# MGI-tech-bioinformatics/SuperPlus

Measured on AMD Instinct MI355X. Metric: k-mers/s (DF createDict stage: trim + canonical k-mer count + solid filter + spectrum + adjacency), higher is better.
Workload: dtype u64

## Files before the change

### superplus_amd/csrc/dfk.hip

```cpp
#include "../../include/dfk.h"
#include "dfk_kernels.h"
#include "dfk_arena.h"

#include <algorithm>
#include <chrono>
#include <cstdarg>
#include <cstdio>
#include <cstdlib>
#include <cstring>
#include <atomic>
#include <fcntl.h>
#include <functional>
#include <new>
#include <string>
#include <sys/mman.h>
#include <sys/stat.h>
#include <unistd.h>
#include <condition_variable>
#include <memory>
#include <mutex>
#include <numeric>
#include <thread>
#include <vector>

// ... 70 lines not shown
    void release(DevBuf& b) { arena.release(b); }
    void shrink(DevBuf& b, size_t keep) { arena.shrink(b, keep); }
    void release_since(uint64_t mark, const DevBuf* keep = nullptr) { arena.release_since(mark, keep); }
    uint64_t largest_allocatable() const { return arena.largest_allocatable(); }
    void drop_empty_chunks() { arena.drop_empty_chunks(); }
    void drop_pool() { arena.drop_pool(); }
    bool have = false;
    uint64_t n_reads = 0;
    struct FileRange { const char* base; uint64_t bytes; int fd; uint64_t off; };
    std::vector<FileRange> file_ranges;
    DevBuf good_len;
    struct Part { DevBuf buf, pre; uint64_t n = 0; uint64_t blist = 0, n_blist = 0; bool listed = false; };
    bool want_blist = false;
    int pending_blist = -1;
    std::function<int()> after_count_launch;
    std::vector<Part> parts;
    uint64_t n_solid = 0, n_boundary = 0;
    unsigned seg_attempt = 0;
    double distinct_per_inst = 0.0;
    double plan_derate = 0.95;
    std::vector<int64_t> hist;
    std::vector<dfk_entry32> sorted, sorted_pre;
    bool sorted_ok = false, sorted_pre_ok = false;
    dfk_stats st{};
    bool shard_open = false, shard_use_bc = false;
    const void* sh_in[7] = {};
    uint64_t sh_packed_bytes = 0, sh_pq_bytes = 0, sh_n_reads = 0, sh_n_inst_local = 0;
    int64_t sh_read_id0 = 0;
    DevBuf shard_send[2];
    uint32_t shard_send_pass[2] = {~0u, ~0u};
// ... 8 lines not shown
    uint32_t shard_world = 1, shard_log2_nb = 0;
    void* shard_state = nullptr;
    void (*shard_state_free)(void*) = nullptr;
    void* lane_pool = nullptr; void (*lane_pool_free)(void*) = nullptr;
    std::mutex lane_mu;
    void* graph_state = nullptr;
    void (*graph_state_free)(void*) = nullptr;
    unsigned int* d_resident = nullptr;
    unsigned int resident_target = 0;
    unsigned int last_wg_idle = 0;
    void* kept[6] = {};
    uint64_t kept_packed_bytes = 0, kept_pq_bytes = 0, kept_n_reads = 0, kept_budget = 0;

    void release_all()
    {
        after_count_launch = nullptr;
        if (stream2) (void)hipStreamSynchronize(stream2);
        DevBuf* live[] = {&good_len, &shard_send[0], &shard_send[1], &shard_recv[0], &shard_recv[1], &adj_keys, &adj_src, &set};
        for (DevBuf* d : live) release(*d);
        for (Part& pt : parts) { release(pt.buf); release(pt.pre); }
        parts.clear();
        arena.reset();
        good_len = shard_send[0] = shard_send[1] = shard_recv[0] = shard_recv[1] = adj_keys = adj_src = set = DevBuf{};
        shard_send_pass[0] = shard_send_pass[1] = ~0u;
        have = false; sorted_ok = sorted_pre_ok = false; sorted.clear(); sorted_pre.clear(); hist.clear();
        n_solid = 0; adj_n = 0; shard_open = false;
        if (shard_state) { shard_state_free(shard_state); shard_state = nullptr; }
        for (void*& p : sh_staged) if (p) { (void)hipFree(p); p = nullptr; }
        budget += budget_taken; budget_taken = 0;
        if (graph_state) { graph_state_free(graph_state); graph_state = nullptr; }
    }
    void drop_kept()
// ... 10 lines not shown
            if (i < 5 && b >= (64ull << 20) && ((uintptr_t)kept[i] & 0xFFF) == 0) arena.adopt(kept[i], b);
            else (void)hipFree(kept[i]);
            kept[i] = nullptr;
        }
        budget += kept_budget; kept_budget = 0; kept_n_reads = 0;
    }
};

namespace {

struct Timer {
    hipEvent_t a{}, b{}; hipStream_t s;
    explicit Timer(hipStream_t st) : s(st) { (void)hipEventCreate(&a); (void)hipEventCreate(&b); }
    ~Timer() { (void)hipEventDestroy(a); (void)hipEventDestroy(b); }
    void start() { (void)hipEventRecord(a, s); }
    float stop() { (void)hipEventRecord(b, s); (void)hipEventSynchronize(b); float ms = 0; (void)hipEventElapsedTime(&ms, a, b); return ms; }
};

template <int K>
int stage_trim(dfk_ctx* c, const Inputs& in, uint64_t* n_inst)
{
    DevBuf ctr; int rc = c->alloc(ctr, 32, "trim counters"); if (rc) return rc;
    HIP_TRY(hipMemsetAsync(ctr.p, 0, 32, c->stream));
    rc = c->alloc(c->good_len, sizeof(uint32_t) * in.n_reads, "goodLens", Place::Low); if (rc) return rc;
    if (in.n_reads) {
        unsigned grid = (unsigned)std::min<uint64_t>((in.n_reads + 255) / 256, 8192);
        hipLaunchKernelGGL(HIP_KERNEL_NAME(k_trim<K>), dim3(grid), dim3(256), 0, c->stream,
                           in.pq, in.pq_off, in.pq_bytes, in.base_off, in.packed_bytes, in.read_len, in.n_reads, c->cfg.min_qual, (uint32_t*)c->good_len.p,
                           (unsigned long long*)ctr.p, (unsigned int*)((char*)ctr.p + 8),
                           (unsigned long long*)((char*)ctr.p + 16));
        HIP_TRY(hipGetLastError());
// ... 337 lines not shown
    return 0;
}

void release_pass(dfk_ctx* c, Partition* P)
{ c->release(P->records); c->release(P->base); c->release(P->ipre); c->release(P->items); }

template <int K> uint64_t item_budget(const dfk_ctx* c)
{
    constexpr uint64_t S = 1ull << CountCfg<K>::LOG2S;
    if (c->cfg.inst_per_item) return c->cfg.inst_per_item;
    if (c->distinct_per_inst <= 0.0) return 3 * S / 2;
    const double b = 0.367 * (double)S / c->distinct_per_inst;
    return (uint64_t)std::min(std::max(b, 0.5 * (double)S), 3.0 * (double)S);
}

struct ScatterJob { Partition P; DevBuf cur, d_bad; hipStream_t st = nullptr; hipEvent_t e0 = nullptr, e1 = nullptr; uint32_t lo = 0, n = 0; };

template <int K>
int scatter_launch(dfk_ctx* c, const Inputs& in, const BucketTable& T, uint32_t log2_world, int64_t read_id0, ScatterJob* J)
{
    const PartParams pp = part_params<K>(c, T.log2_nb, log2_world, read_id0, J->lo, J->n);
    HIP_TRY(hipEventRecord(J->e0, J->st));
    if (in.n_reads)
        hipLaunchKernelGGL(HIP_KERNEL_NAME(k_scatter_runs<K>), dim3((unsigned)((in.n_reads + 256ull * sweep_reads<K>() - 1) / (256ull * sweep_reads<K>()))),
                           dim3(256), 0, J->st,
                           in.packed, in.packed_bytes, in.base_off, (const uint32_t*)c->good_len.p, in.bc,
                           (int64_t)c->cfg.ign_bc_below, in.n_reads, pp, (const uint4*)T.summ.p, (const uint32_t*)T.classes.p,
                           (unsigned long long*)J->cur.p, J->P.n_records, (uint4*)J->P.records.p);
    HIP_TRY(hipGetLastError());
    HIP_TRY(hipEventRecord(J->e1, J->st));
    return 0;
// ... 9 lines not shown
    const uint64_t budget = item_budget<K>(c);
    int rc = pass_tables(c, T.acc, T.log2_nb - log2_world, 1u << log2_world, sub_lo, sub_n, budget, P); if (rc) return rc;
    const uint64_t nb = P->nb;
    rc = c->alloc(J->cur, nb * 8, "bucket cursors"); if (rc) return rc;
    rc = c->alloc(P->records, P->n_records * 32, "super-k-mer records"); if (rc) return rc;
    rc = c->alloc(J->d_bad, 16, "scatter check"); if (rc) return rc;
    HIP_TRY(hipMemcpyAsync(J->cur.p, P->base.p, nb * 8, hipMemcpyDeviceToDevice, c->stream));
    HIP_TRY(hipMemsetAsync(J->d_bad.p, 0, 16, c->stream));
    if (!J->e0) { HIP_TRY(hipEventCreate(&J->e0)); HIP_TRY(hipEventCreate(&J->e1)); }
    (void)pp;
    if (launch_now) return scatter_launch<K>(c, in, T, log2_world, read_id0, J);
    return 0;
}

template <int K>
int scatter_end(dfk_ctx* c, const Inputs& in, const BucketTable& T, uint32_t log2_world, int64_t read_id0, ScatterJob* J)
{
    HIP_TRY(hipEventSynchronize(J->e1));
    float ms = 0; (void)hipEventElapsedTime(&ms, J->e0, J->e1);
    c->st.ms_part_scatter += ms;
    {
        Partition* P = &J->P;
        const PartParams pp = part_params<K>(c, T.log2_nb, log2_world, read_id0, J->lo, J->n);
        const size_t lds_b = sizeof(uint32_t) * pp.W * PART_THREADS + sizeof(uint32_t) * 2 * PART_QCAP * PART_THREADS;
        Timer t(c->stream);
        t.start();
        if (T.n_ovf)
            hipLaunchKernelGGL(HIP_KERNEL_NAME(k_partition<K, true>), dim3((unsigned)((T.n_ovf + PART_THREADS - 1) / PART_THREADS)),
                               dim3(PART_THREADS), lds_b, c->stream,
                               in.packed, in.packed_bytes, in.base_off, (const uint32_t*)c->good_len.p, in.bc,
                               (int64_t)c->cfg.ign_bc_below, in.n_reads, pp, (unsigned long long*)nullptr, (unsigned long long*)nullptr,
                               (unsigned long long*)J->cur.p, P->n_records, (uint4*)P->records.p, (uint4*)nullptr,
                               (const uint32_t*)T.ovf_list.p, T.n_ovf, (const uint64_t*)nullptr, (uint32_t*)nullptr);
        HIP_TRY(hipGetLastError());
        hipLaunchKernelGGL(k_check_cursors, dim3((unsigned)std::min<uint64_t>((P->nb + 255) / 256, 4096)), dim3(256), 0, c->stream, (const unsigned long long*)J->cur.p,
                           (const uint64_t*)P->base.p, P->nb, (unsigned int*)J->d_bad.p);
        HIP_TRY(hipGetLastError());
        c->st.ms_part_scatter += t.stop();
    }
    unsigned int bad = 0;
    HIP_TRY(hipMemcpy(&bad, J->d_bad.p, 4, hipMemcpyDeviceToHost));
    c->release(J->d_bad); c->release(J->cur);
    if (bad) return fail(DFK_E_HIP, "scatter: %u buckets did not receive the records counted for them (run summaries and bucket counters disagree)", bad);
    TRACE("scatter of buckets [%u, %u) done (%llu records, %llu items)", J->lo, J->lo + J->n,
          (unsigned long long)J->P.n_records, (unsigned long long)J->P.n_items);
    return 0;
}

constexpr int E_SPLIT_NO_ROOM = -101;
constexpr int E_SEGMENT_FULL = -100;

struct CountRun {
    CountGlobals* g = nullptr; uint4* seg = nullptr; unsigned long long* hist = nullptr;
    CountParams cp{}; unsigned grid = 0;
    DevBuf big; uint64_t big_cap = 0;
    DevBuf d_hist, d_g;
    DevBuf d_snap;
    DevBuf d_part;
    DevBuf d_wg;
    uint64_t solid_seen = 0, inst_seen = 0;
    uint64_t boundary_seen = 0;
    uint64_t splits_seen = 0;
};

int count_run_begin(dfk_ctx* c, CountRun* R)
{
    int rc = c->alloc(R->d_hist, (uint64_t)HIST_GLOBAL_BINS * 8, "spectrum bins", Place::Low); if (rc) return rc;
    rc = c->alloc(R->d_g, sizeof(CountGlobals), "count globals", Place::Low); if (rc) return rc;
    HIP_TRY(hipMemsetAsync(R->d_hist.p, 0, (uint64_t)HIST_GLOBAL_BINS * 8, c->stream));
    HIP_TRY(hipMemsetAsync(R->d_g.p, 0, sizeof(CountGlobals), c->stream));
    R->g = (CountGlobals*)R->d_g.p; R->hist = (unsigned long long*)R->d_hist.p;
    return c->alloc(R->d_snap, (uint64_t)HIST_GLOBAL_BINS * 8 + 256, "spectrum snapshot", Place::Low);
}

// ... 58 lines not shown
    unsigned long long* ctl = (unsigned long long*)((char*)part.buf.p + part.blist);
    HIP_TRY(hipMemsetAsync(ctl, 0, 16, c->stream2));
    hipLaunchKernelGGL(k_boundary_list, dim3((unsigned)std::min<uint64_t>((part.n + 2047) / 2048, 4096)), dim3(256), 0, c->stream2,
                       (const uint4*)part.buf.p, part.n, (uint32_t*)(ctl + 2), part.n_blist, ctl);
    HIP_TRY(hipGetLastError());
    return 0;
}

template <int K, int NBC>
int launch_count(dfk_ctx* c, const Partition& P, const ItemRange* d_items, uint64_t n_items, const CountRun& R,
                 std::vector<ItemRange>* overflowed, float* kernel_ms, const uint32_t* d_sub = nullptr, bool single_kmer_records = false)
{
    constexpr int LOG2S = CountCfg<K>::LOG2S, NW = CountCfg<K>::NWAVES;
    if (n_items == 0) return 0;
    if (n_items >= (1ull << 32)) return fail(DFK_E_ARG, "too many work items in one pass");
    DevBuf d_ovf;
    int rc = c->alloc(d_ovf, n_items * sizeof(ItemRange), "overflow list"); if (rc) return rc;
    HIP_TRY(hipMemsetAsync(&R.g->next_item, 0, 8, c->stream));
    HIP_TRY(hipMemsetAsync(&R.g->n_wg_idle, 0, 4, c->stream));
    CountParams cp = R.cp; cp.n_items = (uint32_t)n_items; cp.single = single_kmer_records ? 1u : 0u;
    const size_t lds = count_lds_bytes<K, LOG2S, NW, NBC>();
    auto kern = d_sub ? k_count<K, LOG2S, NW, NBC, true> : k_count<K, LOG2S, NW, NBC, false>;
    HIP_TRY(hipFuncSetAttribute(reinterpret_cast<const void*>(kern), hipFuncAttributeMaxDynamicSharedMemorySize, (int)lds));
    TRACE("k_count: %llu items, grid %u, lds %zu, seg_cap %llu", (unsigned long long)n_items, R.grid, lds, (unsigned long long)R.cp.seg_cap);
    Timer tk(c->stream);
    tk.start();
    hipLaunchKernelGGL(kern, dim3(R.grid), dim3(NW * 64), lds, c->stream,
                       (const uint4*)P.records.p, d_items, (const uint64_t*)P.base.p, cp, R.g, R.seg, (WgOut*)R.d_wg.p, R.hist,
                       (ItemRange*)d_ovf.p, d_sub, c->d_resident);
    HIP_TRY(hipGetLastError());
    c->resident_target += R.grid;
    if (c->after_count_launch || c->pending_blist >= 0) {
        hipLaunchKernelGGL(k_gate, dim3(1), dim3(64), 0, c->stream2, (const unsigned int*)c->d_resident, c->resident_target, 200000ull, c->d_resident + 1);
    }
    if (c->after_count_launch) { std::function<int()> f; f.swap(c->after_count_launch); rc = f(); if (rc) return rc; }
    rc = launch_boundary_list(c); if (rc) return rc;
    *kernel_ms += tk.stop();
    CountGlobals g{};
    HIP_TRY(hipMemcpyAsync(&g, R.g, sizeof g, hipMemcpyDeviceToHost, c->stream));
    HIP_TRY(hipStreamSynchronize(c->stream));
    c->last_wg_idle = g.n_wg_idle;
    if (g.n_overflow) {
        const size_t at = overflowed->size();
        overflowed->resize(at + g.n_overflow);
        HIP_TRY(hipMemcpy(overflowed->data() + at, d_ovf.p, sizeof(ItemRange) * g.n_overflow, hipMemcpyDeviceToHost));
    }
    c->release(d_ovf);
    return 0;
}

int gather_diffs(dfk_ctx* c, const std::vector<ItemRange>& ranges, std::initializer_list<std::pair<const DevBuf*, std::vector<uint64_t>*>> tables)
{
    const uint32_t n = (uint32_t)ranges.size();
    DevBuf d_idx, d_val;
    int rc = c->alloc(d_idx, 8ull * n, "gather index"); if (!rc) rc = c->alloc(d_val, 16ull * n, "gather values"); if (rc) return rc;
    HIP_TRY(hipMemcpyAsync(d_idx.p, ranges.data(), 8ull * n, hipMemcpyHostToDevice, c->stream));
    std::vector<uint64_t> val(2 * n);
    for (const auto& t : tables) {
        hipLaunchKernelGGL(k_gather_u64, dim3((2 * n + 255) / 256), dim3(256), 0, c->stream, (const uint64_t*)t.first->p, (const uint32_t*)d_idx.p, 2 * n, (uint64_t*)d_val.p);
        HIP_TRY(hipGetLastError());
        HIP_TRY(hipMemcpyAsync(val.data(), d_val.p, 16ull * n, hipMemcpyDeviceToHost, c->stream));
        HIP_TRY(hipStreamSynchronize(c->stream));
// ... 69 lines not shown
            continue;
        }
        hipLaunchKernelGGL(HIP_KERNEL_NAME(k_big_flags<K, NBC>), dim3(g_slot), dim3(256), 0, c->stream, (const BigItem*)d_items.p,
                           (const uint64_t*)d_slot_pre, n, (uint32_t*)pool.p, cpb, R.g);
        if (cpb.do_adj)
            hipLaunchKernelGGL(HIP_KERNEL_NAME(k_big_resolve<K>), dim3(g_slot), dim3(256), 0, c->stream, (const BigItem*)d_items.p,
                               (const uint64_t*)d_slot_pre, n, (uint32_t*)pool.p);
        hipLaunchKernelGGL(HIP_KERNEL_NAME(k_big_emit<K>), dim3(g_slot), dim3(256), 0, c->stream, (const BigItem*)d_items.p,
                           (const uint64_t*)d_slot_pre, n, (uint32_t*)pool.p, cpb, R.g, (uint4*)R.big.p, R.hist);
        HIP_TRY(hipGetLastError());
        HIP_TRY(hipStreamSynchronize(c->stream));
        c->release(pool);
        break;
    }
    c->release(d_items); c->release(d_fail); c->release(d_pre);
    return 0;
}

template <int K, int NBC>
int count_halved(dfk_ctx* c, const Partition& P, const CountRun& R, bool single_kmer_records, std::vector<ItemRange>& overflowed, std::vector<ItemRange>* singles)
{
    while (!overflowed.empty()) {
        const std::vector<ItemRange> next = halve_items(overflowed, singles);
        overflowed.clear();
        if (next.empty()) break;
        if (!single_kmer_records) TRACE("retrying %zu split items", next.size());
        DevBuf d_next; float ignored = 0;
        int rc = c->alloc(d_next, next.size() * sizeof(ItemRange), "split items"); if (rc) return rc;
        HIP_TRY(hipMemcpyAsync(d_next.p, next.data(), next.size() * sizeof(ItemRange), hipMemcpyHostToDevice, c->stream));
        rc = launch_count<K, NBC>(c, P, (const ItemRange*)d_next.p, next.size(), R, &overflowed, &ignored, nullptr, single_kmer_records);
// ... 74 lines not shown
int barcode_words(const dfk_ctx* c, bool have_bc)
{ return !have_bc ? 0 : (int)std::max<uint32_t>(1, std::min<uint32_t>(c->cfg.min_bc, DFK_MAX_MIN_BC) - (c->cfg.min_bc > 1 ? 1 : 0)); }

template <int K> constexpr uint64_t out_chunk() { return 2ull << CountCfg<K>::LOG2S; }

template <int K>
int count_prepare(dfk_ctx* c, const Partition& P, CountRun& R, int nbc)
{
    const unsigned attempt = c->seg_attempt;
    R.grid = (unsigned)std::max<uint64_t>(1, std::min<uint64_t>(P.n_items, count_grid<K>(c, nbc)));
    uint64_t res = part_entries(P.n_inst, c->cfg.min_freq, R.inst_seen, R.solid_seen);
    res = (res << attempt) + (uint64_t)R.grid * out_chunk<K>();
    const uint64_t room = c->budget > c->held ? (c->budget - c->held) : 0;
    if (res * 32 > room) res = room / 32;
    int rc = c->alloc(R.d_wg, sizeof(WgOut) * R.grid, "workgroup output state"); if (rc) return rc;
    std::vector<WgOut> init(R.grid, WgOut{~0ull, (unsigned int)out_chunk<K>(), 0u});
    HIP_TRY(hipMemcpy(R.d_wg.p, init.data(), sizeof(WgOut) * R.grid, hipMemcpyHostToDevice));
    HIP_TRY(hipMemsetAsync(&R.g->big_cursor, 0, 8, c->stream));
    HIP_TRY(hipMemsetAsync(&R.g->part_cursor, 0, 8, c->stream));
    R.cp = CountParams{c->cfg.min_freq, c->cfg.min_bc, 0, 0, res, c->cfg.min_freq > 1 ? 1u : 0u,
                       (c->cfg.flags & DFK_F_KEEP_PRE_ADJ) ? 1u : 0u};
    R.big_cap = 0;
    rc = c->alloc(R.d_part, std::max<uint64_t>(1, res) * 32, "solid k-mer entries", Place::Low); if (rc) return rc;
    R.seg = (uint4*)R.d_part.p;
    return 0;
}

template <int K>
int finish_part(dfk_ctx* c, const Partition& P, CountRun& R)
{
    CountGlobals hg{};
    std::vector<WgOut> wg(R.grid);
    HIP_TRY(hipMemcpy(&hg, R.d_g.p, sizeof hg, hipMemcpyDeviceToHost));
    HIP_TRY(hipMemcpy(wg.data(), R.d_wg.p, sizeof(WgOut) * R.grid, hipMemcpyDeviceToHost));
    c->release(R.d_wg);
    const uint64_t claimed = hg.part_cursor;
    const HoleMoves mv = plan_hole_moves(wg, out_chunk<K>(), claimed);
    const std::vector<uint64_t>&src = mv.src, &dst = mv.dst; const uint64_t n_lds = mv.n_lds;
    if (hg.solid_overflow || claimed > R.cp.seg_cap || hg.big_cursor > R.big_cap || n_lds + hg.big_cursor > R.cp.seg_cap) {
        c->release(R.big); c->release(R.d_part);
        fail(DFK_E_NOMEM, "the room reserved for a pass's solid k-mers (%llu entries) is full", (unsigned long long)R.cp.seg_cap);
        return E_SEGMENT_FULL;
    }
    if (src.size() != dst.size())
        return fail(DFK_E_HIP, "output compaction: %zu holes, %zu entries to move", dst.size(), src.size());
    dfk_ctx::Part part;
    part.n = n_lds + hg.big_cursor;
    part.buf = R.d_part; R.d_part = DevBuf{};
    if (!src.empty()) {
        DevBuf d_mv; int rc = c->alloc(d_mv, 16ull * src.size(), "hole moves"); if (rc) return rc;
        HIP_TRY(hipMemcpyAsync(d_mv.p, src.data(), 8ull * src.size(), hipMemcpyHostToDevice, c->stream));
        HIP_TRY(hipMemcpyAsync((uint64_t*)d_mv.p + src.size(), dst.data(), 8ull * src.size(), hipMemcpyHostToDevice, c->stream));
        hipLaunchKernelGGL(k_fill_holes, dim3((unsigned)((src.size() + 255) / 256)), dim3(256), 0, c->stream, (uint4*)part.buf.p,
                           (const uint64_t*)d_mv.p, (const uint64_t*)d_mv.p + src.size(), (uint64_t)src.size());
        HIP_TRY(hipGetLastError());
        HIP_TRY(hipStreamSynchronize(c->stream));
        c->release(d_mv);
    }
    if (hg.big_cursor)
        HIP_TRY(hipMemcpyAsync((char*)part.buf.p + 32 * n_lds, R.big.p, 32 * hg.big_cursor, hipMemcpyDeviceToDevice, c->stream));
    HIP_TRY(hipStreamSynchronize(c->stream));
    c->release(R.big);
    const uint64_t nb_part = hg.n_boundary - R.boundary_seen;
    R.boundary_seen = hg.n_boundary;
    c->st.n_overflow_items += hg.n_split - R.splits_seen;
    R.splits_seen = hg.n_split;
    uint64_t keep = part.n * 32;
    part.listed = c->want_blist && nb_part == 0;
    if (c->want_blist && nb_part && keep + 16 + 4 * nb_part <= part.buf.bytes && part.n < (1ull << 32)) {
        part.blist = keep; part.n_blist = nb_part; part.listed = true;
        keep += 16 + 4 * nb_part;
    }
    c->shrink(part.buf, keep);
    c->parts.push_back(part);
    if (part.blist) c->pending_blist = (int)c->parts.size() - 1;
    c->n_solid += part.n; c->st.n_solid = c->n_solid;
// ... 99 lines not shown
            HIP_TRY(hipMemcpyAsync(pt.pre.p, pt.buf.p, pt.n * 32, hipMemcpyDeviceToDevice, c->stream));
    }
    HIP_TRY(hipGetLastError());
    return 0;
}

template <int K>
int stage_adjacency(dfk_ctx* c)
{
    Timer t(c->stream);
    t.start();
    int rc = make_pre_view(c); if (rc) return rc;
    if (c->cfg.min_freq > 1 && c->n_solid && c->n_boundary) {
        bool listed = c->want_blist;
        for (const dfk_ctx::Part& pt : c->parts) listed = listed && pt.listed;
        if (c->want_blist) {
            rc = launch_boundary_list(c); if (rc) return rc;
            HIP_TRY(hipStreamSynchronize(c->stream2));
        }
        if (listed) {
            uint64_t total = 0;
            for (const dfk_ctx::Part& pt : c->parts) {
                if (!pt.blist) continue;
                unsigned long long ctl[2] = {0, 0};
                HIP_TRY(hipMemcpy(ctl, (const char*)pt.buf.p + pt.blist, 16, hipMemcpyDeviceToHost));
                if (ctl[1] || ctl[0] != pt.n_blist)
                    return fail(DFK_E_HIP, "boundary list: %llu entries listed, the count kernels reported %llu", ctl[0], (unsigned long long)pt.n_blist);
                total += pt.n_blist;
            }
            if (total != c->n_boundary) listed = false;
        }
        if (!listed) { rc = build_set(c); if (rc) return rc; }
        else {
            uint64_t slots = 1ull << std::max<uint32_t>(10, ceil_log2(2 * c->n_boundary + 2));
            rc = c->alloc(c->set, slots * sizeof(SetSlot), "boundary k-mer set"); if (rc) return rc;
            c->set_mask = slots - 1;
            hipLaunchKernelGGL(k_fill_u64, dim3(2048), dim3(256), 0, c->stream, (uint64_t*)c->set.p, slots * 2, ~0ull);
            for (const dfk_ctx::Part& pt : c->parts)
                if (pt.n_blist)
                    hipLaunchKernelGGL(k_set_insert_list, dim3((unsigned)((pt.n_blist + 255) / 256)), dim3(256), 0, c->stream, (const uint4*)pt.buf.p,
                                       (const uint32_t*)((const char*)pt.buf.p + pt.blist + 16), pt.n_blist, (SetSlot*)c->set.p, c->set_mask);
            HIP_TRY(hipGetLastError());
        }
        DevBuf d_n; rc = c->alloc(d_n, 16, "probe counter"); if (rc) return rc;
        HIP_TRY(hipMemsetAsync(d_n.p, 0, 16, c->stream));
        for (const dfk_ctx::Part& pt : c->parts) {
            if (!pt.n) continue;
            if (listed) {
                if (pt.n_blist)
                    hipLaunchKernelGGL(HIP_KERNEL_NAME(k_adjacency_list<K>), dim3((unsigned)std::min<uint64_t>((pt.n_blist + 255) / 256, 16384)), dim3(256), 0,
                                       c->stream, (uint4*)pt.buf.p, (const uint32_t*)((const char*)pt.buf.p + pt.blist + 16), pt.n_blist,
                                       (const SetSlot*)c->set.p, c->set_mask, (unsigned long long*)d_n.p);
// ... 66 lines not shown
    const uint32_t forced = (uint32_t)c->cfg.reserved[0];
    const uint32_t per_forced = forced ? std::max<uint32_t>(1, (sub_nb + forced - 1) / forced) : 0;
    const bool overlap = getenv("DFK_NO_OVERLAP") == nullptr;
    uint32_t n_passes = 0, retries = 0;
    c->seg_attempt = 0; c->distinct_per_inst = 0.0;
    struct Job { ScatterJob sj; Arena::PassBlock blk; uint64_t mark = 0; bool valid = false; };
    Job cur, nxt;
    auto drop_events = [&](Job& j) { if (j.sj.e0) { (void)hipEventDestroy(j.sj.e0); (void)hipEventDestroy(j.sj.e1); j.sj.e0 = j.sj.e1 = nullptr; } };
    static const double defer_below = getenv("DFK_DEFER_SWEEP_BELOW") ? atof(getenv("DFK_DEFER_SWEEP_BELOW")) : 1.0;
    auto start = [&](Job& j, uint32_t lo, uint32_t n, bool may_defer = false) -> int {
        j.sj = ScatterJob{}; j.mark = c->alloc_seq; j.valid = false;
        const bool defer = may_defer && (double)n < defer_below * (double)sub_nb;
        TRACE("pass range [%u, %u) of %u (%.1f %%), %.2f GB held of %.2f", lo, lo + n, sub_nb, 100.0 * n / sub_nb, c->held / 1e9, c->budget / 1e9);
        j.blk = Arena::PassBlock{};
        int r = c->alloc(j.blk.block, pass_block_bytes(n, sub_nb, T.n_records), "pass block");
        if (!r) { Arena::Current in_blk(c->arena, j.blk); StreamSwap sw(c, c->stream2); r = scatter_begin<K>(c, in, T, 0, 0, lo, n, &j.sj, !defer); }
        if (r) { (void)hipStreamSynchronize(c->stream2); c->release_since(j.mark); drop_events(j); return r; }
        if (defer) { ScatterJob* sj = &j.sj; c->after_count_launch = [c, &in, &T, sj]() { return scatter_launch<K>(c, in, T, 0, 0, sj); }; TRACE("  (its sweep starts behind k_count)"); }
        j.valid = true;
        return 0;
    };
    auto start_alone = [&](Job& j, uint32_t lo) -> int {
        for (;;) {
            const uint32_t n = forced ? std::min(per_forced, sub_nb - lo) : plan_range(plan_inputs(c, T, R, sub_nb, lo, overlap), c->arena.free_blocks(), nullptr);
            if (!forced && n < sub_nb - lo && (uint64_t)n * 1024 < sub_nb)
                return fail(DFK_E_NOMEM, "HBM budget too small: %.2f GB free of %.2f GB allows passes of %u of %u buckets",
                            (c->budget - c->held) / 1e9, c->budget / 1e9, n, sub_nb);
            const int r = start(j, lo, n);
            if (r != DFK_E_NOMEM || forced || n <= 16 || ++retries > 12) return r;
            c->plan_derate *= 0.7;
            TRACE("out of HBM (%s): planning smaller passes", g_err.c_str());
        }
    };
// ... 2 lines not shown
        const uint32_t lo = cur.sj.lo, n = cur.sj.n, nlo = lo + n;
        rc = scatter_end<K>(c, in, T, 0, 0, &cur.sj); if (rc) return rc;
        const dfk_stats st0 = c->st;
        rc = count_snapshot(c, &R, false); if (rc) return rc;
        { Arena::Current in_blk(c->arena, cur.blk); rc = count_prepare<K>(c, cur.sj.P, R, barcode_words(c, in.bc != nullptr)); }
        nxt.valid = false;
        if (!rc && overlap && nlo < sub_nb) {
            const Partition& P = cur.sj.P;
            (void)P;
            const RunningPass rp{cur.blk.block.bytes, cur.sj.P.n_inst, n, c->arena.offset_of(cur.blk.block)};
            const uint32_t n2 = forced ? std::min(per_forced, sub_nb - nlo) : plan_range(plan_inputs(c, T, R, sub_nb, nlo, overlap), c->arena.free_blocks(), &rp);
            if (n2) {
                const int r2 = start(nxt, nlo, n2, true);
                if (r2 && r2 != DFK_E_NOMEM) return r2;
            }
        }
        if (!rc) rc = count_run_nbc<K>(c, cur.sj.P, R, barcode_words(c, in.bc != nullptr));
        if (c->after_count_launch) {
            std::function<int()> f; f.swap(c->after_count_launch);
            if (!rc) { const int r3 = f(); if (r3) return r3; } else nxt.valid = false;
        }
        if (rc == DFK_E_NOMEM || rc == E_SEGMENT_FULL) {
            HIP_TRY(hipStreamSynchronize(c->stream)); HIP_TRY(hipStreamSynchronize(c->stream2));
            c->release_since(cur.mark);
            R.d_wg = R.big = R.d_part = DevBuf{};
            drop_events(cur); drop_events(nxt); nxt.valid = false;
            int rc2 = count_snapshot(c, &R, true); if (rc2) return rc2;
            const float ms_scatter = c->st.ms_part_scatter, ms_count = c->st.ms_count, ms_fb = c->st.ms_fallback;
            c->st = st0;
            c->st.ms_part_scatter = ms_scatter; c->st.ms_count = ms_count; c->st.ms_fallback = ms_fb;
            if (++retries > 12) return DFK_E_NOMEM;
            if (rc == E_SEGMENT_FULL) { ++c->seg_attempt; TRACE("the room reserved for the pass's solid k-mers was too small: redoing the pass with twice as much"); }
            else if (forced || n <= 16) return rc;
            else { c->plan_derate *= 0.7; TRACE("out of HBM (%s): redoing the pass smaller", g_err.c_str()); }
            rc = start_alone(cur, lo); if (rc) return rc;
            continue;
        }
        if (rc) return rc;
        release_pass(c, &cur.sj.P);
        c->release(cur.blk.block);
// ... 351 lines not shown
        TRACE("hbm_budget_bytes %.1f GB is more than 90 %% of the free HBM: clamped to %.1f GB", cfg->hbm_budget_bytes / 1e9, cap / 1e9);
    *out = c;
    return 0;
    });
}

void dfk_destroy(dfk_ctx* c)
{
    if (!c) return;
    (void)hipSetDevice(c->device);
    c->release_all();
    c->drop_kept();
    c->drop_pool();
    if (c->lane_pool) { c->lane_pool_free(c->lane_pool); c->lane_pool = nullptr; }
    if (c->d_resident) (void)hipFree(c->d_resident);
    if (c->stream) (void)hipStreamDestroy(c->stream);
    if (c->stream2) (void)hipStreamDestroy(c->stream2);
    delete c;
}

int dfk_count_device(dfk_ctx* c, const void* d_packed, uint64_t packed_bytes, const void* d_base_off,
                     const void* d_read_len, const void* d_pq, uint64_t pq_nbytes, const void* d_pq_off,
                     const void* d_bc, uint64_t n_reads)
{
    return guarded([&]() -> int {
    if (!c) return fail(DFK_E_ARG, "null context");
    if (n_reads && (!d_packed || !d_base_off || !d_read_len || !d_pq || !d_pq_off)) return fail(DFK_E_ARG, "null input array");
    if (n_reads >= (1ull << 32)) return fail(DFK_E_ARG, "more than 2^32-1 reads in one shard");
    HIP_TRY(hipSetDevice(c->device));
    c->release_all();
// ... 297 lines not shown
```

### superplus_amd/csrc/dfk_kernels.h

```cpp
#pragma once
#include <type_traits>
#include "dfk_device.h"
#include "dfk_fallback.h"

namespace dfk {

template <int K>
__global__ void __launch_bounds__(256)
k_trim(const uint8_t* __restrict__ pq, const uint64_t* __restrict__ pq_off, uint64_t pq_nbytes,
       const uint64_t* __restrict__ base_off, uint64_t packed_bytes, const uint32_t* __restrict__ read_len,
       uint64_t n_reads, uint32_t min_qual, uint32_t* __restrict__ good_len,
       unsigned long long* __restrict__ n_inst, unsigned int* __restrict__ bad,
       unsigned long long* __restrict__ sum_good)
{
    unsigned long long mine = 0, good = 0;
    bool any_bad = false;
    for (uint64_t r = (uint64_t)blockIdx.x * blockDim.x + threadIdx.x; r < n_reads; r += (uint64_t)gridDim.x * blockDim.x) {
        uint32_t gl = 0;
        uint64_t p = pq_off[r], end = pq_off[r + 1];
        uint32_t idx = 0, run = 0;
        const uint64_t b0 = base_off[r], b1 = base_off[r + 1];
        bool ok = p <= end && end <= pq_nbytes && b0 <= b1 && b1 <= packed_bytes && b1 - b0 >= ((uint64_t)read_len[r] + 3) / 4;
        if (!ok) end = p;
        while (p < end) {
// ... 1522 lines not shown
        if (!items_done) atomicAdd(&g->n_wg_idle, 1u);
    }
}

__global__ void __launch_bounds__(64)
k_gate(const unsigned int* __restrict__ ctr, unsigned int target, unsigned long long max_ticks, unsigned int* __restrict__ timed_out)
{
    if (threadIdx.x != 0) return;
    const unsigned long long t0 = wall_clock64();
    while ((int)(__hip_atomic_load(ctr, __ATOMIC_RELAXED, __HIP_MEMORY_SCOPE_AGENT) - target) < 0) {
        if (wall_clock64() - t0 > max_ticks) { __hip_atomic_fetch_add(timed_out, 1u, __ATOMIC_RELAXED, __HIP_MEMORY_SCOPE_AGENT); break; }
        __builtin_amdgcn_s_sleep(64);
    }
}

template <int K, int LOG2S, int NWAVES, int NBC>
constexpr size_t count_lds_bytes()
{
    return sizeof(uint32_t) * ((size_t)(KTraits<K>::KW + 3 + (NBC > 1 ? NBC - 1 : 0)) * (1u << LOG2S) + COUNT_HIST_BINS + CTL_N + (1u << LOG2S) / 2 + (1u << LOG2S) / 2) + sizeof(WaveStage<K>) * NWAVES;
}

template <int K, int NWAVES, int NBC>
__global__ void __launch_bounds__(NWAVES * 64)
k_big_insert(const uint4* __restrict__ records, const BigItem* __restrict__ items, const uint64_t* __restrict__ rec_base,
             const uint64_t* __restrict__ chunk_pre, uint32_t n_items, uint32_t* __restrict__ tab_pool,
             unsigned long long* __restrict__ ticket, uint32_t* __restrict__ failed)
{
    constexpr int KW = KTraits<K>::KW;
    __shared__ WaveStage<K> stages[NWAVES];
    __shared__ uint32_t fill, ovf;
// ... 735 lines not shown
```

Measured before the change: 64.78 billion.

## Cut host syncs and transfers around count passes with pinned read-back buffers

Measured after the change: 63.90 billion. -1.4%, worse.

```diff
diff --git a/superplus_amd/csrc/dfk.hip b/superplus_amd/csrc/dfk.hip
--- a/superplus_amd/csrc/dfk.hip
+++ b/superplus_amd/csrc/dfk.hip
@@ -108,6 +108,23 @@
     bool want_blist = false;
     int pending_blist = -1;
     std::function<int()> after_count_launch;
+    std::function<int(hipEvent_t)> under_count;
+    struct Pinned {
+        void* p = nullptr; size_t bytes = 0;
+        int reserve(size_t n)
+        {
+            if (n <= bytes) return 0;
+            if (p) (void)hipHostFree(p);
+            p = nullptr; bytes = 0;
+            n = (n + 0xFFFF) & ~(size_t)0xFFFF;
+            if (hipHostMalloc(&p, n, hipHostMallocDefault) != hipSuccess) { p = nullptr; return fail(DFK_E_NOMEM, "no pinned host memory (%zu bytes)", n); }
+            bytes = n;
+            return 0;
+        }
+        void drop() { if (p) (void)hipHostFree(p); p = nullptr; bytes = 0; }
+    } pin, mv;
+    hipEvent_t ev_fill = nullptr; bool fill_queued = false;
+    uint32_t count_attr_set = 0;
     std::vector<Part> parts;
     uint64_t n_solid = 0, n_boundary = 0;
     unsigned seg_attempt = 0;
@@ -146,8 +163,10 @@
 
     void release_all()
     {
-        after_count_launch = nullptr;
+        after_count_launch = nullptr; under_count = nullptr;
         if (stream2) (void)hipStreamSynchronize(stream2);
+        if (fill_queued) { (void)hipEventSynchronize(ev_fill); fill_queued = false; }
+        pending_blist = -1;
         DevBuf* live[] = {&good_len, &shard_send[0], &shard_send[1], &shard_recv[0], &shard_recv[1], &adj_keys, &adj_src, &set};
         for (DevBuf* d : live) release(*d);
         for (Part& pt : parts) { release(pt.buf); release(pt.pre); }
@@ -188,7 +207,9 @@
     explicit Timer(hipStream_t st) : s(st) { (void)hipEventCreate(&a); (void)hipEventCreate(&b); }
     ~Timer() { (void)hipEventDestroy(a); (void)hipEventDestroy(b); }
     void start() { (void)hipEventRecord(a, s); }
-    float stop() { (void)hipEventRecord(b, s); (void)hipEventSynchronize(b); float ms = 0; (void)hipEventElapsedTime(&ms, a, b); return ms; }
+    float stop() { mark(); return wait(); }
+    void mark() { (void)hipEventRecord(b, s); }
+    float wait() { (void)hipEventSynchronize(b); float ms = 0; (void)hipEventElapsedTime(&ms, a, b); return ms; }
 };
 
 template <int K>
@@ -556,7 +577,14 @@
     return (uint64_t)std::min(std::max(b, 0.5 * (double)S), 3.0 * (double)S);
 }
 
-struct ScatterJob { Partition P; DevBuf cur, d_bad; hipStream_t st = nullptr; hipEvent_t e0 = nullptr, e1 = nullptr; uint32_t lo = 0, n = 0; };
+constexpr size_t COUNT_READBACK_MISC = 64, COUNT_READBACK_WG = 128;
+static_assert(sizeof(CountGlobals) <= COUNT_READBACK_MISC, "the read-back buffer's layout");
+inline size_t count_readback_bytes(unsigned grid) { return COUNT_READBACK_WG + sizeof(WgOut) * (size_t)grid; }
+
+struct ScatterJob {
+    Partition P; DevBuf cur, d_bad; hipStream_t st = nullptr; hipEvent_t e0 = nullptr, e1 = nullptr; uint32_t lo = 0, n = 0;
+    bool checked = false; unsigned int bad = 0; float ms_checks = 0;
+};
 
 template <int K>
 int scatter_launch(dfk_ctx* c, const Inputs& in, const BucketTable& T, uint32_t log2_world, int64_t read_id0, ScatterJob* J)
@@ -596,32 +624,42 @@
 }
 
 template <int K>
+int scatter_checks(dfk_ctx* c, const Inputs& in, const BucketTable& T, uint32_t log2_world, int64_t read_id0, ScatterJob* J, hipStream_t st)
+{
+    Partition* P = &J->P;
+    const PartParams pp = part_params<K>(c, T.log2_nb, log2_world, read_id0, J->lo, J->n);
+    const size_t lds_b = sizeof(uint32_t) * pp.W * PART_THREADS + sizeof(uint32_t) * 2 * PART_QCAP * PART_THREADS;
+    int rc = c->pin.reserve(COUNT_READBACK_WG); if (rc) return rc;
+    unsigned int* const h_bad = (unsigned int*)((char*)c->pin.p + COUNT_READBACK_MISC);
+    Timer t(st);
+    t.start();
+    if (T.n_ovf)
+        hipLaunchKernelGGL(HIP_KERNEL_NAME(k_partition<K, true>), dim3((unsigned)((T.n_ovf + PART_THREADS - 1) / PART_THREADS)),
+                           dim3(PART_THREADS), lds_b, st,
+                           in.packed, in.packed_bytes, in.base_off, (const uint32_t*)c->good_len.p, in.bc,
+                           (int64_t)c->cfg.ign_bc_below, in.n_reads, pp, (unsigned long long*)nullptr, (unsigned long long*)nullptr,
+                           (unsigned long long*)J->cur.p, P->n_records, (uint4*)P->records.p, (uint4*)nullptr,
+                           (const uint32_t*)T.ovf_list.p, T.n_ovf, (const uint64_t*)nullptr, (uint32_t*)nullptr);
+    HIP_TRY(hipGetLastError());
+    hipLaunchKernelGGL(k_check_cursors, dim3((unsigned)std::min<uint64_t>((P->nb + 255) / 256, 4096)), dim3(256), 0, st, (const unsigned long long*)J->cur.p,
+                       (const uint64_t*)P->base.p, P->nb, (unsigned int*)J->d_bad.p);
+    HIP_TRY(hipGetLastError());
+    t.mark();
+    HIP_TRY(hipMemcpyAsync(h_bad, J->d_bad.p, 4, hipMemcpyDeviceToHost, st));
+    HIP_TRY(hipStreamSynchronize(st));
+    J->ms_checks = t.wait(); J->bad = *h_bad; J->checked = true;
+    return 0;
+}
+
+template <int K>
 int scatter_end(dfk_ctx* c, const Inputs& in, const BucketTable& T, uint32_t log2_world, int64_t read_id0, ScatterJob* J)
 {
     HIP_TRY(hipEventSynchronize(J->e1));
     float ms = 0; (void)hipEventElapsedTime(&ms, J->e0, J->e1);
     c->st.ms_part_scatter += ms;
-    {
-        Partition* P = &J->P;
-        const PartParams pp = part_params<K>(c, T.log2_nb, log2_world, read_id0, J->lo, J->n);
-        const size_t lds_b = sizeof(uint32_t) * pp.W * PART_THREADS + sizeof(uint32_t) * 2 * PART_QCAP * PART_THREADS;
-        Timer t(c->stream);
-        t.start();
-        if (T.n_ovf)
-            hipLaunchKernelGGL(HIP_KERNEL_NAME(k_partition<K, true>), dim3((unsigned)((T.n_ovf + PART_THREADS - 1) / PART_THREADS)),
-                               dim3(PART_THREADS), lds_b, c->stream,
-                               in.packed, in.packed_bytes, in.base_off, (const uint32_t*)c->good_len.p, in.bc,
-                               (int64_t)c->cfg.ign_bc_below, in.n_reads, pp, (unsigned long long*)nullptr, (unsigned long long*)nullptr,
-                               (unsigned long long*)J->cur.p, P->n_records, (uint4*)P->records.p, (uint4*)nullptr,
-                               (const uint32_t*)T.ovf_list.p, T.n_ovf, (const uint64_t*)nullptr, (uint32_t*)nullptr);
-        HIP_TRY(hipGetLastError());
-        hipLaunchKernelGGL(k_check_cursors, dim3((unsigned)std::min<uint64_t>((P->nb + 255) / 256, 4096)), dim3(256), 0, c->stream, (const unsigned long long*)J->cur.p,
-                           (const uint64_t*)P->base.p, P->nb, (unsigned int*)J->d_bad.p);
-        HIP_TRY(hipGetLastError());
-        c->st.ms_part_scatter += t.stop();
-    }
-    unsigned int bad = 0;
-    HIP_TRY(hipMemcpy(&bad, J->d_bad.p, 4, hipMemcpyDeviceToHost));
+    if (!J->checked) { const int rc = scatter_checks<K>(c, in, T, log2_world, read_id0, J, c->stream); if (rc) return rc; }
+    c->st.ms_part_scatter += J->ms_checks;
+    const unsigned int bad = J->bad;
     c->release(J->d_bad); c->release(J->cur);
     if (bad) return fail(DFK_E_HIP, "scatter: %u buckets did not receive the records counted for them (run summaries and bucket counters disagree)", bad);
     TRACE("scatter of buckets [%u, %u) done (%llu records, %llu items)", J->lo, J->lo + J->n,
@@ -640,6 +678,9 @@
     DevBuf d_snap;
     DevBuf d_part;
     DevBuf d_wg;
+    mutable DevBuf d_ovf;
+    mutable bool zeroed = false;
+    mutable bool read_back = false;
     uint64_t solid_seen = 0, inst_seen = 0;
     uint64_t boundary_seen = 0;
     uint64_t splits_seen = 0;
@@ -728,38 +769,52 @@
     constexpr int LOG2S = CountCfg<K>::LOG2S, NW = CountCfg<K>::NWAVES;
     if (n_items == 0) return 0;
     if (n_items >= (1ull << 32)) return fail(DFK_E_ARG, "too many work items in one pass");
-    DevBuf d_ovf;
-    int rc = c->alloc(d_ovf, n_items * sizeof(ItemRange), "overflow list"); if (rc) return rc;
-    HIP_TRY(hipMemsetAsync(&R.g->next_item, 0, 8, c->stream));
-    HIP_TRY(hipMemsetAsync(&R.g->n_wg_idle, 0, 4, c->stream));
+    int rc = 0;
+    if (R.d_ovf.bytes < n_items * sizeof(ItemRange)) {
+        c->release(R.d_ovf);
+        rc = c->alloc(R.d_ovf, n_items * sizeof(ItemRange), "overflow list"); if (rc) return rc;
+    }
+    rc = c->pin.reserve(count_readback_bytes(R.grid)); if (rc) return rc;
+    if (!R.zeroed) {
+        hipLaunchKernelGGL(k_count_init, dim3(1), dim3(64), 0, c->stream, (WgOut*)nullptr, 0u, 0u, R.g, 0);
+        HIP_TRY(hipGetLastError());
+    }
+    R.zeroed = false;
     CountParams cp = R.cp; cp.n_items = (uint32_t)n_items; cp.single = single_kmer_records ? 1u : 0u;
     const size_t lds = count_lds_bytes<K, LOG2S, NW, NBC>();
     auto kern = d_sub ? k_count<K, LOG2S, NW, NBC, true> : k_count<K, LOG2S, NW, NBC, false>;
-    HIP_TRY(hipFuncSetAttribute(reinterpret_cast<const void*>(kern), hipFuncAttributeMaxDynamicSharedMemorySize, (int)lds));
+    const uint32_t attr_bit = 1u << (2 * NBC + (d_sub ? 1 : 0));
+    if (!(c->count_attr_set & attr_bit)) {
+        HIP_TRY(hipFuncSetAttribute(reinterpret_cast<const void*>(kern), hipFuncAttributeMaxDynamicSharedMemorySize, (int)lds));
+        c->count_attr_set |= attr_bit;
+    }
     TRACE("k_count: %llu items, grid %u, lds %zu, seg_cap %llu", (unsigned long long)n_items, R.grid, lds, (unsigned long long)R.cp.seg_cap);
     Timer tk(c->stream);
     tk.start();
     hipLaunchKernelGGL(kern, dim3(R.grid), dim3(NW * 64), lds, c->stream,
                        (const uint4*)P.records.p, d_items, (const uint64_t*)P.base.p, cp, R.g, R.seg, (WgOut*)R.d_wg.p, R.hist,
-                       (ItemRange*)d_ovf.p, d_sub, c->d_resident);
-    HIP_TRY(hipGetLastError());
+                       (ItemRange*)R.d_ovf.p, d_sub, c->d_resident);
+    HIP_TRY(hipGetLastError());
+    tk.mark();
+    CountGlobals* const hg = (CountGlobals*)c->pin.p;
+    HIP_TRY(hipMemcpyAsync(hg, R.g, sizeof(CountGlobals), hipMemcpyDeviceToHost, c->stream));
+    HIP_TRY(hipMemcpyAsync((char*)c->pin.p + COUNT_READBACK_WG, R.d_wg.p, sizeof(WgOut) * R.grid, hipMemcpyDeviceToHost, c->stream));
     c->resident_target += R.grid;
     if (c->after_count_launch || c->pending_blist >= 0) {
         hipLaunchKernelGGL(k_gate, dim3(1), dim3(64), 0, c->stream2, (const unsigned int*)c->d_resident, c->resident_target, 200000ull, c->d_resident + 1);
     }
     if (c->after_count_launch) { std::function<int()> f; f.swap(c->after_count_launch); rc = f(); if (rc) return rc; }
     rc = launch_boundary_list(c); if (rc) return rc;
-    *kernel_ms += tk.stop();
-    CountGlobals g{};
-    HIP_TRY(hipMemcpyAsync(&g, R.g, sizeof g, hipMemcpyDeviceToHost, c->stream));
+    if (c->under_count) { std::function<int(hipEvent_t)> f; f.swap(c->under_count); rc = f(tk.b); if (rc) return rc; }
+    *kernel_ms += tk.wait();
     HIP_TRY(hipStreamSynchronize(c->stream));
-    c->last_wg_idle = g.n_wg_idle;
-    if (g.n_overflow) {
+    R.read_back = true;
+    c->last_wg_idle = hg->n_wg_idle;
+    if (hg->n_overflow) {
         const size_t at = overflowed->size();
-        overflowed->resize(at + g.n_overflow);
-        HIP_TRY(hipMemcpy(overflowed->data() + at, d_ovf.p, sizeof(ItemRange) * g.n_overflow, hipMemcpyDeviceToHost));
-    }
-    c->release(d_ovf);
+        overflowed->resize(at + hg->n_overflow);
+        HIP_TRY(hipMemcpy(overflowed->data() + at, R.d_ovf.p, sizeof(ItemRange) * hg->n_overflow, hipMemcpyDeviceToHost));
+    }
     return 0;
 }
 
@@ -859,6 +914,7 @@
         break;
     }
     c->release(d_items); c->release(d_fail); c->release(d_pre);
+    R.read_back = false;
     return 0;
 }
 
@@ -963,10 +1019,9 @@
     const uint64_t room = c->budget > c->held ? (c->budget - c->held) : 0;
     if (res * 32 > room) res = room / 32;
     int rc = c->alloc(R.d_wg, sizeof(WgOut) * R.grid, "workgroup output state"); if (rc) return rc;
-    std::vector<WgOut> init(R.grid, WgOut{~0ull, (unsigned int)out_chunk<K>(), 0u});
-    HIP_TRY(hipMemcpy(R.d_wg.p, init.data(), sizeof(WgOut) * R.grid, hipMemcpyHostToDevice));
-    HIP_TRY(hipMemsetAsync(&R.g->big_cursor, 0, 8, c->stream));
-    HIP_TRY(hipMemsetAsync(&R.g->part_cursor, 0, 8, c->stream));
+    hipLaunchKernelGGL(k_count_init, dim3((R.grid + 255) / 256), dim3(256), 0, c->stream, (WgOut*)R.d_wg.p, R.grid, (unsigned int)out_chunk<K>(), R.g, 1);
+    HIP_TRY(hipGetLastError());
+    R.zeroed = true; R.read_back = false;
     R.cp = CountParams{c->cfg.min_freq, c->cfg.min_bc, 0, 0, res, c->cfg.min_freq > 1 ? 1u : 0u,
                        (c->cfg.flags & DFK_F_KEEP_PRE_ADJ) ? 1u : 0u};
     R.big_cap = 0;
@@ -978,10 +1033,17 @@
 template <int K>
 int finish_part(dfk_ctx* c, const Partition& P, CountRun& R)
 {
-    CountGlobals hg{};
-    std::vector<WgOut> wg(R.grid);
-    HIP_TRY(hipMemcpy(&hg, R.d_g.p, sizeof hg, hipMemcpyDeviceToHost));
-    HIP_TRY(hipMemcpy(wg.data(), R.d_wg.p, sizeof(WgOut) * R.grid, hipMemcpyDeviceToHost));
+    c->release(R.d_ovf);
+    if (!R.read_back) {
+        int rc = c->pin.reserve(count_readback_bytes(R.grid)); if (rc) return rc;
+        HIP_TRY(hipMemcpyAsync(c->pin.p, R.d_g.p, sizeof(CountGlobals), hipMemcpyDeviceToHost, c->stream));
+        HIP_TRY(hipMemcpyAsync((char*)c->pin.p + COUNT_READBACK_WG, R.d_wg.p, sizeof(WgOut) * R.grid, hipMemcpyDeviceToHost, c->stream));
+        HIP_TRY(hipStreamSynchronize(c->stream));
+    }
+    R.read_back = false;
+    const CountGlobals hg = *(const CountGlobals*)c->pin.p;
+    const WgOut* const wg0 = (const WgOut*)((const char*)c->pin.p + COUNT_READBACK_WG);
+    const std::vector<WgOut> wg(wg0, wg0 + R.grid);
     c->release(R.d_wg);
     const uint64_t claimed = hg.part_cursor;
     const HoleMoves mv = plan_hole_moves(wg, out_chunk<K>(), claimed);
@@ -997,18 +1059,21 @@
     part.n = n_lds + hg.big_cursor;
     part.buf = R.d_part; R.d_part = DevBuf{};
     if (!src.empty()) {
-        DevBuf d_mv; int rc = c->alloc(d_mv, 16ull * src.size(), "hole moves"); if (rc) return rc;
-        HIP_TRY(hipMemcpyAsync(d_mv.p, src.data(), 8ull * src.size(), hipMemcpyHostToDevice, c->stream));
-        HIP_TRY(hipMemcpyAsync((uint64_t*)d_mv.p + src.size(), dst.data(), 8ull * src.size(), hipMemcpyHostToDevice, c->stream));
+        if (c->fill_queued) { HIP_TRY(hipEventSynchronize(c->ev_fill)); c->fill_queued = false; }
+        int rc = c->mv.reserve(16ull * src.size()); if (rc) return rc;
+        uint64_t* mv = (uint64_t*)c->mv.p;
+        memcpy(mv, src.data(), 8ull * src.size()); memcpy(mv + src.size(), dst.data(), 8ull * src.size());
         hipLaunchKernelGGL(k_fill_holes, dim3((unsigned)((src.size() + 255) / 256)), dim3(256), 0, c->stream, (uint4*)part.buf.p,
-                           (const uint64_t*)d_mv.p, (const uint64_t*)d_mv.p + src.size(), (uint64_t)src.size());
+                           (const uint64_t*)mv, (const uint64_t*)mv + src.size(), (uint64_t)src.size());
         HIP_TRY(hipGetLastError());
-        HIP_TRY(hipStreamSynchronize(c->stream));
-        c->release(d_mv);
+        if (!c->ev_fill) HIP_TRY(hipEventCreateWithFlags(&c->ev_fill, hipEventDisableTiming));
+        HIP_TRY(hipEventRecord(c->ev_fill, c->stream));
+        c->fill_queued = true;
+        if (c->stream2) HIP_TRY(hipStreamWaitEvent(c->stream2, c->ev_fill, 0));
     }
     if (hg.big_cursor)
         HIP_TRY(hipMemcpyAsync((char*)part.buf.p + 32 * n_lds, R.big.p, 32 * hg.big_cursor, hipMemcpyDeviceToDevice, c->stream));
-    HIP_TRY(hipStreamSynchronize(c->stream));
+    if (hg.big_cursor || !c->want_blist) HIP_TRY(hipStreamSynchronize(c->stream));
     c->release(R.big);
     const uint64_t nb_part = hg.n_boundary - R.boundary_seen;
     R.boundary_seen = hg.n_boundary;
@@ -1138,28 +1203,46 @@
     if (c->cfg.min_freq > 1 && c->n_solid && c->n_boundary) {
         bool listed = c->want_blist;
         for (const dfk_ctx::Part& pt : c->parts) listed = listed && pt.listed;
+        const uint64_t slots = 1ull << std::max<uint32_t>(10, ceil_log2(2 * c->n_boundary + 2));
+        rc = c->alloc(c->set, slots * sizeof(SetSlot), "boundary k-mer set"); if (rc) return rc;
+        c->set_mask = slots - 1;
+        hipLaunchKernelGGL(k_fill_u64, dim3(2048), dim3(256), 0, c->stream, (uint64_t*)c->set.p, slots * 2, ~0ull);
+        HIP_TRY(hipGetLastError());
         if (c->want_blist) {
             rc = launch_boundary_list(c); if (rc) return rc;
+        }
+        if (listed) {
+            size_t n_lists = 0;
+            for (const dfk_ctx::Part& pt : c->parts) n_lists += pt.blist ? 1 : 0;
+            rc = c->pin.reserve(24 * n_lists + 64); if (rc) return rc;
+            const unsigned long long** h_ptr = (const unsigned long long**)c->pin.p;
+            unsigned long long* h_ctl = (unsigned long long*)((char*)c->pin.p + 8 * n_lists);
+            size_t k = 0;
+            for (const dfk_ctx::Part& pt : c->parts) if (pt.blist) h_ptr[k++] = (const unsigned long long*)((const char*)pt.buf.p + pt.blist);
+            if (n_lists) {
+                hipLaunchKernelGGL(k_gather_ctl, dim3((unsigned)((2 * n_lists + 63) / 64)), dim3(64), 0, c->stream2, (const unsigned long long* const*)h_ptr, (unsigned int)n_lists, h_ctl);
+                HIP_TRY(hipGetLastError());
+            }
             HIP_TRY(hipStreamSynchronize(c->stream2));
-        }
-        if (listed) {
-            uint64_t total = 0;
+            uint64_t total = 0; k = 0;
             for (const dfk_ctx::Part& pt : c->parts) {
                 if (!pt.blist) continue;
-                unsigned long long ctl[2] = {0, 0};
-                HIP_TRY(hipMemcpy(ctl, (const char*)pt.buf.p + pt.blist, 16, hipMemcpyDeviceToHost));
-                if (ctl[1] || ctl[0] != pt.n_blist)
+                const unsigned long long* ctl = h_ctl + 2 * k++;
+                if (ctl[1] || ctl[0] != pt.n_blist) {
+                    c->release(c->set);
                     return fail(DFK_E_HIP, "boundary list: %llu entries listed, the count kernels reported %llu", ctl[0], (unsigned long long)pt.n_blist);
+                }
                 total += pt.n_blist;
             }
             if (total != c->n_boundary) listed = false;
-        }
-        if (!listed) { rc = build_set(c); if (rc) return rc; }
-        else {
-            uint64_t slots = 1ull << std::max<uint32_t>(10, ceil_log2(2 * c->n_boundary + 2));
-            rc = c->alloc(c->set, slots * sizeof(SetSlot), "boundary k-mer set"); if (rc) return rc;
-            c->set_mask = slots - 1;
-            hipLaunchKernelGGL(k_fill_u64, dim3(2048), dim3(256), 0, c->stream, (uint64_t*)c->set.p, slots * 2, ~0ull);
+        } else if (c->want_blist) HIP_TRY(hipStreamSynchronize(c->stream2));
+        if (!listed) {
+            for (const dfk_ctx::Part& pt : c->parts)
+                if (pt.n)
+                    hipLaunchKernelGGL(k_set_insert, dim3((unsigned)((pt.n + 255) / 256)), dim3(256), 0, c->stream,
+                                       (const uint4*)pt.buf.p, pt.n, (SetSlot*)c->set.p, c->set_mask);
+            HIP_TRY(hipGetLastError());
+        } else {
             for (const dfk_ctx::Part& pt : c->parts)
                 if (pt.n_blist)
                     hipLaunchKernelGGL(k_set_insert_list, dim3((unsigned)((pt.n_blist + 255) / 256)), dim3(256), 0, c->stream, (const uint4*)pt.buf.p,
@@ -1256,9 +1339,23 @@
         TRACE("pass range [%u, %u) of %u (%.1f %%), %.2f GB held of %.2f", lo, lo + n, sub_nb, 100.0 * n / sub_nb, c->held / 1e9, c->budget / 1e9);
         j.blk = Arena::PassBlock{};
         int r = c->alloc(j.blk.block, pass_block_bytes(n, sub_nb, T.n_records), "pass block");
-        if (!r) { Arena::Current in_blk(c->arena, j.blk); StreamSwap sw(c, c->stream2); r = scatter_begin<K>(c, in, T, 0, 0, lo, n, &j.sj, !defer); }
+        auto begin = [c, &in, &T, &j, lo, n]() -> int {
+            Arena::Current in_blk(c->arena, j.blk); StreamSwap sw(c, c->stream2);
+            return scatter_begin<K>(c, in, T, 0, 0, lo, n, &j.sj);
+        };
+        if (!r && !defer) r = begin();
         if (r) { (void)hipStreamSynchronize(c->stream2); c->release_since(j.mark); drop_events(j); return r; }
-        if (defer) { ScatterJob* sj = &j.sj; c->after_count_launch = [c, &in, &T, sj]() { return scatter_launch<K>(c, in, T, 0, 0, sj); }; TRACE("  (its sweep starts behind k_count)"); }
+        if (defer) {
+            c->after_count_launch = [c, &j, &drop_events, begin]() -> int {
+                const uint64_t mark2 = c->alloc_seq;
+                const int r2 = begin();
+                if (!r2) return 0;
+                (void)hipStreamSynchronize(c->stream2); c->release_since(mark2); c->release(j.blk.block); drop_events(j);
+                j.valid = false;
+                return r2 == DFK_E_NOMEM ? 0 : r2;
+            };
+            TRACE("  (its tables and its sweep start behind k_count)");
+        }
         j.valid = true;
         return 0;
     };
@@ -1291,8 +1388,20 @@
                 const int r2 = start(nxt, nlo, n2, true);
                 if (r2 && r2 != DFK_E_NOMEM) return r2;
             }
+            if (nxt.valid)
+                c->under_count = [c, &in, &T, &nxt](hipEvent_t count_done) -> int {
+                    if (!nxt.valid || !nxt.sj.e1) return 0;
+                    for (;;) {
+                        const bool swept = hipEventQuery(nxt.sj.e1) == hipSuccess, counted = !swept && hipEventQuery(count_done) == hipSuccess;
+                        (void)hipGetLastError();
+                        if (swept) return scatter_checks<K>(c, in, T, 0, 0, &nxt.sj, c->stream2);
+                        if (counted) return 0;
+                        std::this_thread::sleep_for(std::chrono::microseconds(50));
+                    }
+                };
         }
         if (!rc) rc = count_run_nbc<K>(c, cur.sj.P, R, barcode_words(c, in.bc != nullptr));
+        c->under_count = nullptr;
         if (c->after_count_launch) {
             std::function<int()> f; f.swap(c->after_count_launch);
             if (!rc) { const int r3 = f(); if (r3) return r3; } else nxt.valid = false;
@@ -1300,7 +1409,7 @@
         if (rc == DFK_E_NOMEM || rc == E_SEGMENT_FULL) {
             HIP_TRY(hipStreamSynchronize(c->stream)); HIP_TRY(hipStreamSynchronize(c->stream2));
             c->release_since(cur.mark);
-            R.d_wg = R.big = R.d_part = DevBuf{};
+            R.d_wg = R.big = R.d_part = R.d_ovf = DevBuf{};
             drop_events(cur); drop_events(nxt); nxt.valid = false;
             int rc2 = count_snapshot(c, &R, true); if (rc2) return rc2;
             const float ms_scatter = c->st.ms_part_scatter, ms_count = c->st.ms_count, ms_fb = c->st.ms_fallback;
@@ -1682,6 +1791,8 @@
     c->drop_pool();
     if (c->lane_pool) { c->lane_pool_free(c->lane_pool); c->lane_pool = nullptr; }
     if (c->d_resident) (void)hipFree(c->d_resident);
+    c->pin.drop(); c->mv.drop();
+    if (c->ev_fill) (void)hipEventDestroy(c->ev_fill);
     if (c->stream) (void)hipStreamDestroy(c->stream);
     if (c->stream2) (void)hipStreamDestroy(c->stream2);
     delete c;
diff --git a/superplus_amd/csrc/dfk_kernels.h b/superplus_amd/csrc/dfk_kernels.h
--- a/superplus_amd/csrc/dfk_kernels.h
+++ b/superplus_amd/csrc/dfk_kernels.h
@@ -1560,6 +1560,25 @@
     }
 }
 
+__global__ void __launch_bounds__(256)
+k_count_init(WgOut* __restrict__ wg, unsigned int n_wg, unsigned int chunk, CountGlobals* __restrict__ g, int new_pass)
+{
+    const unsigned int i = blockIdx.x * blockDim.x + threadIdx.x;
+    if (new_pass)
+        for (unsigned int j = i; j < n_wg; j += gridDim.x * blockDim.x) wg[j] = WgOut{~0ull, chunk, 0u};
+    if (i == 0) {
+        g->next_item = 0; g->n_overflow = 0; g->n_wg_idle = 0;
+        if (new_pass) { g->big_cursor = 0; g->part_cursor = 0; }
+    }
+}
+
+__global__ void __launch_bounds__(64)
+k_gather_ctl(const unsigned long long* const* __restrict__ ctl, unsigned int n, unsigned long long* __restrict__ out)
+{
+    const unsigned int i = blockIdx.x * blockDim.x + threadIdx.x;
+    if (i < 2 * n) out[i] = ctl[i >> 1][i & 1];
+}
+
 template <int K, int LOG2S, int NWAVES, int NBC>
 constexpr size_t count_lds_bytes()
 {
```
